# AdrianHeath988/orion

Hardware: AMD Instinct MI355X
Metric: encrypted images/sec (LoLa N=2^15) + NTT HBM GB/s vs peak (higher is better)
Workload: dtype u64; 1 GPU; LoLA (models/lola.py) lola_n15: N=2^15, LogQ=[60]+[40]x11, LogP=[60,60], input level 5, Standard ring; batch_per_gpu=64, global_batch=64

## Files before the change

orion_amd/csrc/backend.hip:

```cpp
#include <hip/hip_runtime.h>
#include <math.h>
#include <string.h>

#include <algorithm>
#include <atomic>
#include <map>
#include <memory>
#include <mutex>
#include <set>
#include <shared_mutex>
#include <stdexcept>
#include <string>
#include <thread>
#include <unordered_map>
#include <vector>
#include <complex>

#include "../../include/orion_hip.h"
#include "common.h"
#include "hostmath.h"
#include "wire.h"

int orion_launch_ntt(int logN, const LimbSet& s, const DeviceTables* tb, bool inverse, hipStream_t st);
int orion_launch_ntt_io(int logN, const NttIO& io, const DeviceTables* tb, bool inverse, hipStream_t st);
int orion_launch_ntt2(int logN, const NttIO& io, const DeviceTables* tb, bool inverse, hipStream_t st);
int orion_launch_ntt2s(int logN, const NttIO& io, const DeviceTables* tb, bool inverse, hipStream_t st,
                       bool rows_only = false);
int orion_ntt_init();
int orion_launch_ew(int op, const LimbSet& o, const LimbSet& a, const LimbSet& b, const u64* s, const u64* ss,
                    const DeviceTables* tb, int N, hipStream_t st);
int orion_launch_tensor(const LimbSet& d, const LimbSet& a, const LimbSet& b, const DeviceTables* tb, int N,
                        hipStream_t st);
int orion_launch_gather(u64* dst, long long d_comp, long long d_limb, int nimg, int nlimb, const GatherTable& T,
                        int N, hipStream_t st);
int orion_launch_basis_ext(const LimbSet& out, const LimbSet& in, const BasisExtTable* T, const DeviceTables* tb,
                           int N, hipStream_t st);
int orion_launch_modup_all(const LimbSet& D, const LimbSet& in, const BasisExtTable* Ts, int beta, int K,
                           int nqp, const DeviceTables* tb, int N, hipStream_t st);
int orion_launch_ks_mac(const LimbSet& out, const LimbSet& D, const LimbSet& own, const MacGroups& G, int ngroup,
                        int beta, const DeviceTables* tb, int N, hipStream_t st);
int orion_launch_automorph(const LimbSet& o, const LimbSet& a, const u32* idx, const DeviceTables* tb, int N,
                           int accumulate, hipStream_t st);
int orion_launch_lt_bsgs(const LimbSet& t0, const LimbSet& t1, const LimbSet& D, const LimbSet& ct,
                         const LtBabies& Bb, const LtPlan* plan, int g0, int g1, int accumulate, const LimbSet& ptl,
                         const DeviceTables* tb, int N, hipStream_t st);
int orion_launch_lt_giant(const LimbSet& acc, const LimbSet& D, const LimbSet& own, const LimbSet& t0,
                          const LimbSet& z, const LtGiants& G, const DeviceTables* tb, int N, hipStream_t st);

int orion_launch_encode(const float* vals, int nvals, int B, double2* v, const double2* tw_inv, int logn, bool ci,
                        const LimbSet& out, double scale, const DeviceTables* tb, hipStream_t st);
int orion_launch_decode(const LimbSet& x, const u64* garner, double scale, int logn, bool ci, double2* v,
// ... 267 lines not shown
  long long limb_stride() const { return (long long)B * N; }
  long long comp_stride() const { return (long long)nlimb * B * N; }
};

struct EvKey {
  Poly k;
  int level = 0;
};

struct Ciphertext {
  Poly poly;
  int level = 0;
  long double scale = 1;
  std::string poison;
  std::shared_ptr<char> share;
};

struct Plaintext {
  Poly poly;
  int level = 0;
  long double scale = 1;
  bool qp = false;
};

struct LinTrans {
  int level = 0, N1 = 1;
  float ratio = 1;
  std::vector<int> idx;
  std::map<int, Plaintext> diags;
  std::map<int, Poly> sdiags;
// ... 35 lines not shown
  }
  static Hook& hook() {
    static Hook h = nullptr;
    return h;
  }
  using Hold = void (*)(const T&);
  static Hold& hold() {
    static Hold h = nullptr;
    return h;
  }
  using Check = void (*)(const T&);
  static Check& check() {
    static Check c = nullptr;
    return c;
  }
  int add(T&& v) {
    std::lock_guard<std::mutex> lk(mu_);
    int id;
    if (!free_.empty()) {
      id = *free_.begin();
      free_.erase(free_.begin());
    } else {
      id = next_++;
    }
    map_[id] = Entry{std::make_unique<T>(std::move(v)), g_birth.fetch_add(1), false};
    if (born) born->insert(id);
    return id;
  }
  std::set<int>* born = nullptr;
  T& get(int id) {
    const int own = id >> kCtxShift;
    if (id >= 0 && own != (base_ >> kCtxShift)) {
      HandlePool* o = resolver() ? resolver()(own) : nullptr;
      if (!o || o == this) throw std::runtime_error("handle not found: " + std::to_string(id));
      unsigned long long birth = 0;
      T& v = o->get_local(id, &birth, true);
      if (check()) check()(v);
      if (hook()) hook()(own, birth);
      if (hold()) hold()(v);
      return v;
    }
    T& v = get_local(id, nullptr);
    if (check()) check()(v);
    return v;
  }
  void touch(int id) {
    const int own = id >> kCtxShift;
    HandlePool* o = this;
    if (id >= 0 && own != (base_ >> kCtxShift)) o = resolver() ? resolver()(own) : nullptr;
    if (!o) throw std::runtime_error("handle not found: " + std::to_string(id));
    std::lock_guard<std::mutex> lk(o->mu_);
    auto it = o->map_.find(id);
    if (it != o->map_.end()) it->second.birth = g_birth.fetch_add(1);
// ... 106 lines not shown
  DeviceTables* d_tb = nullptr;
  std::vector<void*> static_bufs;
  double2 *tw_inv = nullptr, *tw_fwd = nullptr;
  std::map<int, u64*> garner;
  Prng prng{0x0123456789abcdefull};
  EncSampler enc_sampler;

  Poly sk, pk, rlk;
  bool have_sk = false, have_pk = false, have_rlk = false;
  std::map<u64, EvKey> gks;
  std::map<u64, int> key_hint;
  std::map<u64, u32*> autidx;
  std::map<std::pair<int, int>, BasisExtTable*> betab;
  std::map<std::pair<int, int>, std::vector<int>> betab_pos;
  std::map<int, BasisExtTable*> modup_arr;

  HandlePool<Plaintext> pts;
  HandlePool<Ciphertext> cts;
  HandlePool<LinTrans> lts;

  struct GraphRec {
    hipGraph_t g = nullptr;
    hipGraphExec_t x = nullptr;
    std::vector<std::pair<void*, size_t>> pins;
    std::vector<std::shared_ptr<void>> holds;
  };
  std::set<int> capture_born;
  std::vector<std::shared_ptr<void>> capture_holds;
  std::map<int, GraphRec> graphs;
  int next_graph = 0;
// ... 15 lines not shown
      if (gr) hipGraphDestroy(gr);
    }
    for (auto& kv : graphs) {
      hipGraphExecDestroy(kv.second.x);
      hipGraphDestroy(kv.second.g);
    }
    graphs.clear();
    gks.clear();
    sk = pk = rlk = Poly();
    pts.reset();
    cts.reset();
    lts.reset();
    for (auto& kv : autidx) hipFree(kv.second);
    for (auto& kv : betab) hipFree(kv.second);
    for (auto& kv : modup_arr) hipFree(kv.second);
    for (auto& kv : garner) hipFree(kv.second);
    for (void* p : static_bufs) hipFree(p);
    if (d_tb) hipFree(d_tb);
    for (auto& r : prof_recs) {
      hipEventDestroy(r.e0);
      hipEventDestroy(r.e1);
    }
    for (auto e : ev_free) hipEventDestroy(e);
    if (own_stream && stream) hipStreamDestroy(stream);
  }

  hipEvent_t ev() {
    if (!ev_free.empty()) {
      hipEvent_t e = ev_free.back();
      ev_free.pop_back();
// ... 557 lines not shown
    }
    const u128 two64 = (u128)1 << 64;
    if (src32 && t < (1ull << 32) && (ssum + 1) * t < ((u128)1 << 63)) return BEXT_NARROW;
    if (!bext_modes) return BEXT_LAZY;
    if (ns >= 3 && src32 && t >= (1ull << 32) && t < (1ull << 61) && ssum * M30 < two64 &&
        ssum * T1 < (u128)4 * t * t)
      return BEXT_WT;
    if (ns >= 4 && src62 && t < (1ull << 31) && (u128)(ns + 1) * M30 * T1 < two64 && ssum * T1 < ((u128)1 << 96))
      return BEXT_NT;
    return BEXT_LAZY;
  }

  BasisExtTable* make_betab(const std::vector<int>& src, const std::vector<int>& dst, bool centered = false) {
    no_capture("a basis extension table");
    BasisExtTable T;
    memset(&T, 0, sizeof(T));
    T.ns = (int)src.size();
    T.nt = (int)dst.size();
    T.centered = centered && T.ns == 1 ? 1 : 0;
    T.chalf = mods[src[0]] >> 1;
    if (T.ns > ORION_MAXSRC || T.nt > ORION_MAXLIMB) throw std::runtime_error("basis extension too large");
    for (int i = 0; i < T.ns; ++i) {
      const u64 si = mods[src[i]];
      T.src_mod[i] = src[i];
      T.sq[i] = si;
      T.qhatinv[i] = hm_invmod(prod_mod(src, i, si), si);
      T.qhatinv_s[i] = hm_shoup(T.qhatinv[i], si);
      T.qf[i] = (double)si;
      T.qinv_f[i] = 1.0 / T.qf[i];
    }
// ... 11 lines not shown
      R.nSs = hm_shoup(R.nS, tm);
      for (int v = 0; v < 3; ++v) R.vS[v] = hm_mulmod((u64)v, R.nS, tm);
      R.qd = (double)tm;
      R.tinv = 1.0 / (double)tm;
      R.tinv32 = std::ldexp(R.tinv, 32);
      R.k = 64 - __builtin_clzll(tm);
      R.mu2 = R.k <= 61 ? (u64)(((u128)1 << (2 * R.k + 2)) / tm) : 0;
      R.c64 = (u64)(((u128)1 << 64) % tm);
      auto pieces = [](u64 x, u32& a, u32& b, u32& c) {
        a = (u32)(x & 0x3fffffffu), b = (u32)((x >> 30) & 0x3fffffffu), c = (u32)(x >> 60);
      };
      for (int i = 0; i < T.ns; ++i) pieces(R.qh[i], R.h0[i], R.h1[i], R.h2[i]);
      pieces(R.nS, R.n0, R.n1, R.n2);
      R.mode = T.centered ? BEXT_LAZY : bext_mode(src, T.ns, tm);
    }
    BasisExtTable* d;
    HIPCHK(hipMalloc(&d, sizeof(T)));
    h2d(d, &T, sizeof(T));
    return d;
  }
  BasisExtTable* modup_tab(int level, int digit, std::vector<int>& tpos) {
    auto key = std::make_pair(level, digit);
    auto it = betab.find(key);
    if (it != betab.end()) {
      tpos = betab_pos[key];
      return it->second;
    }
    const int lo = digit * K, hi = std::min((digit + 1) * K, level + 1);
    std::vector<int> src = iota(lo, hi), dst;
    tpos.clear();
    for (int j = 0; j <= level + K; ++j) {
      if (j >= lo && j < hi) continue;
      tpos.push_back(j);
      dst.push_back(qp_mod(level, j));
// ... 14 lines not shown
    for (int i = 0; i < beta; ++i)
      HIPCHK(hipMemcpyAsync(d + i, modup_tab(level, i, tpos), sizeof(BasisExtTable), hipMemcpyDeviceToDevice,
                             stream));
    HIPCHK(hipStreamSynchronize(stream));
    modup_arr[level] = d;
    return d;
  }
  BasisExtTable* moddown_tab(int level) {
    auto key = std::make_pair(level, -1);
    auto it = betab.find(key);
    if (it != betab.end()) return it->second;
    std::vector<int> src;
    for (int k = 0; k < K; ++k) src.push_back(L + k);
    BasisExtTable* d = make_betab(src, iota(0, level + 1));
    betab[key] = d;
    return d;
  }

  u64 galois_element(int k) const {
    return hm_powmod(5, (u64)(long long)k & (nthroot - 1), nthroot);
  }
  const u32* aut_index(u64 g) {
    auto it = autidx.find(g);
    if (it != autidx.end()) return it->second;
    no_capture("an automorphism index table");
    std::vector<u32> idx(N);
    const int logM = logN + (ci ? 1 : 0);
    const u64 mask = nthroot - 1;
    for (int j = 0; j < N; ++j) {
      const u64 t1 = 2 * hm_bitrev(j, logM) + 1;
// ... 394 lines not shown
      if (rows_done) throw std::runtime_error("moddown: rows pass done, but the fused path is not taken");
      ntt(xp, true);
      Poly ext = alloc(nc, level + 1, B);
      LimbSet le = lsq(ext, 0, nc, level);
      {
        Scope sc(this, P_BEXT, 8.0 * N * B * nc * (K + level + 1));
        if (orion_launch_basis_ext(le, xp, moddown_tab(level), d_tb, N, stream))
          throw std::runtime_error("basis_ext: unsupported source count");
      }
      NttIO io = nio(dst, le);
      epilogue(io);
      ntt_io(io, false);
    }
    if (aut_g && !scatter) automorph(out, dst, aut_g, aut_acc);
  }
  void keyswitch(const LimbSet& c, int level, int B, const Poly& key, int klvl, const Poly& out,
                 const u64* add0 = nullptr, const u64* add1 = nullptr, u64 aut_g = 0, bool aut_acc = false) {
    if (klvl < level) throw std::runtime_error("evaluation key made for a lower level");
    Poly u = alloc(2, level + 1 + K, B);
    const bool rows_q = mac_fwd_rows && moddown_rows_fusable(lsqp(u, 0, 2, level, level), level,
                                                             lsq(out, 0, 2, level), aut_g, aut_acc);
    bool fwd_rows = false;
    Poly D = decompose(c, level, B, rows_q, &fwd_rows);
    const int beta = (level + 1 + K - 1) / K;
    const LimbSet uq = lsqp(u, 0, 2, level, level), oq = lsq(out, 0, 2, level);
    const bool rows = moddown_rows_fusable(uq, level, oq, aut_g, aut_acc);
    mac_groups(uq, 0, lsqp(D, 0, beta, level, level), 0, c, 0, {key.ptr()}, {klvl}, beta, add0, 0,
               add0 ? level + 1 : 0, add1, rows ? level + 1 : 0, fwd_rows);
    moddown(uq, level, oq, aut_g, aut_acc, rows);
  }
  std::vector<u64> p_mod_q(int level) const {
    std::vector<u64> v;
    for (int j = 0; j <= level; ++j) {
      u64 P = 1;
      for (int k = 0; k < K; ++k) P = hm_mulmod(P, mods[L + k] % mods[j], mods[j]);
      v.push_back(P);
    }
    return v;
  }

  Ciphertext new_ct(int level, int B, long double scale) {
    Ciphertext c;
    c.poly = alloc(2, level + 1, B);
    c.level = level;
    c.scale = scale;
    return c;
  }
  Ciphertext clone(const Ciphertext& a) {
    Ciphertext c = new_ct(a.level, a.poly.B, a.scale);
    copy(lsq(c.poly, 0, 2, a.level), lsq(a.poly, 0, 2, a.level));
    return c;
  }
  void gather(Ciphertext& dst, const std::vector<GatherSrc>& src) {
    const int nl = dst.level + 1;
    const Poly& D = dst.poly;
    if ((int)src.size() != D.B || D.nlimb < nl) throw std::runtime_error("gather: destination shape mismatch");
    for (int b0 = 0; b0 < D.B; b0 += ORION_MAXGATHER) {
      const int n = std::min(ORION_MAXGATHER, D.B - b0);
      GatherTable T;
      memset(&T, 0, sizeof(T));
      for (int i = 0; i < n; ++i) T.src[i] = src[b0 + i];
// ... 26 lines not shown
      io.s[j] = hm_invmod(mods[l] % mods[j], mods[j]);
      io.ss[j] = hm_shoup(io.s[j], mods[j]);
    }
    (void)B;
    intt_then_fwd(nio(last, last), io, 1);
    ct.level = l - 1;
    ct.scale /= (long double)mods[l];
  }

  int batch_of(int a, int b) const {
    if (a == b || b == 1) return a;
    if (a == 1) return b;
    throw std::runtime_error("batch size mismatch");
  }

  Ciphertext mul_relin(const Ciphertext& a, const Ciphertext& b) {
    if (!have_rlk) throw std::runtime_error("relinearization key not generated");
    const int level = std::min(a.level, b.level);
    const int B = batch_of(a.poly.B, b.poly.B);
    Poly d = alloc(3, level + 1, B);
    {
      LimbSet ld = lsq(d, 0, 3, level);
      const bool square = a.poly.ptr() == b.poly.ptr();
      Scope sc(this, P_TENSOR, 8.0 * N * (level + 1) * B * (square ? 5 : 7));
      orion_launch_tensor(ld, lsq(a.poly, 0, 2, level, B), lsq(b.poly, 0, 2, level, B), d_tb, N, stream);
    }
    Ciphertext out = new_ct(level, B, a.scale * b.scale);
    keyswitch(lsq(d, 2, 1, level), level, B, rlk, L - 1, out.poly, d.ptr(), d.ptr() + d.comp_stride());
    return out;
  }

  Ciphertext rotate(const Ciphertext& a, int k) { return apply_galois(a, galois_element(k)); }
  void rotate_into(const Ciphertext& a, int k, Ciphertext& out) {
    const u64 g = galois_element(k);
    const int level = a.level, B = a.poly.B;
    const EvKey& key = galois_key(g, level);
    if (!out.poly.buf) out.poly = new_ct(level, B, a.scale).poly;
    out.level = level;
    keyswitch(lsq(a.poly, 1, 1, level), level, B, key.k, key.level, out.poly, a.poly.ptr(), nullptr, g);
  }
// ... 94 lines not shown
    }
    h2d(T.d_plan, plans.data(), nplan * sizeof(LtPlan));
    T.n_plan = nplan;
    T.plan_dirty = false;
  }
  void build_dirty_plans() {
    for (int id : lts.live()) {
      LinTrans& T = lts.get(id);
      if (!T.plan_dirty || T.giants.empty()) continue;
      bool all = true;
      for (int d : T.idx) all = all && T.diags.count(d & (slots - 1));
      if (all) build_plan(T);
    }
  }

  Ciphertext eval_lt(LinTrans& T, const Ciphertext& ct) {
    const int level = std::min(ct.level, T.level);
    const int B = ct.poly.B, nqp = level + 1 + K;
    const int beta = (level + 1 + K - 1) / K;
    if (T.giants.empty()) throw std::runtime_error("linear transform without diagonals");
    for (int d : T.idx)
      if (!T.diags.count(d & (slots - 1)))
        throw std::runtime_error("linear transform diagonal " + std::to_string(d) +
                                 " is not loaded (io_mode load: call LoadPlaintextDiagonal first)");
    if (T.plan_dirty) build_plan(T);
    const std::vector<u64> pq = p_mod_q(level);
    const int nb = (int)T.slots.size();
    const int nzb = nb - (T.slots.back() == 0 ? 1 : 0);

    Poly D = nzb > 0 ? decompose(lsq(ct.poly, 1, 1, level), level, B) : alloc(1, 1, 1);
    LimbSet dl = lsqp(D, 0, 1, level, level);
// ... 37 lines not shown
          for (int gi = p * LT_MAXG; gi < p * LT_MAXG + gcount; ++gi)
            for (int b : T.index.at(T.gorder[gi]))
              for (int s = 0; s < Bb.nb; ++s)
                if (T.slots[s0 + s] == b) ++npair;
          Scope sc(this, P_LTMAC,
                   8.0 * N * (rows * ((nzb ? beta : 0) + 2.0 + 2.0 * gcount * (s0 ? 2 : 1)) +
                              (double)nqp * (2.0 * beta * nrot + npair)));
          if (orion_launch_lt_bsgs(t0, t1, dl, ctl, Bb, T.d_plan + p, 0, gcount, s0 > 0, ptl, d_tb, N, stream))
            throw std::runtime_error("lt_bsgs launch failed");
        }
      }
    }

    Poly acc = alloc(2, nqp, B);
    LimbSet la = lsqp(acc, 0, 2, level, level);
    Ciphertext out = new_ct(level, B, ct.scale * (long double)mods[T.level]);
    const LimbSet lo = lsq(out.poly, 0, 2, level);
    const bool rows = nzg > 0 && nzg <= ORION_MAXGROUP && moddown_rows_fusable(la, level, lo, 0, false);
    LimbSet z = lsqp(Tt, ng - 1, 2, level, level);
    z.comp_stride = (long long)ng * Tt.comp_stride();
    if (nzg > 0) {
      Poly T1q = alloc(nzg, level + 1, B);
      moddown(lsqp(Tt, ng, nzg, level, level), level, lsq(T1q, 0, nzg, level));
      Poly Dg = decompose(lsq(T1q, 0, nzg, level), level, B);
      for (int g0 = 0; g0 < nzg; g0 += ORION_MAXGROUP) {
        LtGiants G;
        memset(&G, 0, sizeof(G));
        G.ng = std::min(ORION_MAXGROUP, nzg - g0);
        G.beta = beta;
        G.K = K;
        G.level = level;
        G.L = L;
        G.has_zero = (has_g0 && g0 == 0) ? 1 : 0;
// ... 17 lines not shown
        Poly part;
        if (g0 > 0) {
          part = alloc(2, nqp, B);
          a = lsqp(part, 0, 2, level, level);
        }
        const double rows = (double)nqp * B;
        Scope sc(this, P_LTGIANT, 8.0 * N * (rows * (G.ng * (beta + 1.0) + 2.0 + 2.0 * G.has_zero) +
                                          (double)nqp * 2.0 * beta * G.ng));
        if (orion_launch_lt_giant(a, dg, own, t0, z, G, d_tb, N, stream))
          throw std::runtime_error("lt_giant launch failed");
        if (g0 > 0) ew(EW_ADD, la, la, a);
      }
    } else {
      copy(la, z);
    }
    moddown(la, level, lo, 0, false, rows);
    return out;
  }

  Plaintext encode_dev(const float* dvals, int nvals, int B, int level, long double scale, bool qp) {
    const int n = slots;
    if (nvals > n) throw std::runtime_error("too many values for the slot count");
    std::vector<int> md = iota(0, level + 1);
    if (qp)
      for (int k = 0; k < K; ++k) md.push_back(L + k);
    const int nl = (int)md.size();
    Plaintext pt;
    pt.level = level;
    pt.scale = scale;
    pt.qp = qp;
    pt.poly = alloc(1, nl, B);
// ... 575 lines not shown
    if (!bt.d2s.k.buf || !bt.s2d.k.buf) gen_circuit_keys(bt);
    for (const KeyNeed& n : bt.need)
      if (n.kind == BK_GALOIS) gen_galois(n.gel, n.level);
    HIPCHK(hipStreamSynchronize(stream));
  }

  Ciphertext mul_i(const Bootstrapper& bt, const Ciphertext& a) {
    Ciphertext o = new_ct(a.level, a.poly.B, a.scale);
    LimbSet mi = ls(bt.mono_i, 0, 1, iota(0, a.level + 1), iota(0, a.level + 1), a.poly.B);
    mi.ncomp = 2;
    mi.comp_stride = 0;
    ew(EW_MUL, lsq(o.poly, 0, 2, a.level), lsq(a.poly, 0, 2, a.level), mi);
    return o;
  }
  Ciphertext lt_rescale(LinTrans& T, const Ciphertext& x) {
    Ciphertext y = eval_lt(T, x);
    rescale_inplace(y);
    y.scale = x.scale;
    return y;
  }
  Ciphertext eval_mod(const Bootstrapper& bt, const Ciphertext& u) {
    Ciphertext y = eval_poly(u, bt.cosp, bt.t0);
    for (int k = 0; k < bt.r; ++k) {
      Ciphertext t = mul_relin(y, y);
      const LimbSet lt = lsq(t.poly, 0, 2, t.level);
      ew(EW_ADD, lt, lt, lt);
      std::vector<u64> c = big_const_residues(-bt.dac[k] * t.scale, t.level);
      ew1(EW_ADDC, lsq(t.poly, 0, 1, t.level), lsq(t.poly, 0, 1, t.level), &c);
      rescale_inplace(t);
      y = std::move(t);
    }
    return y;
// ... 150 lines not shown
  HIPCHK(hipStreamWaitEvent(me.stream, e, 0));
  HIPCHK(hipEventDestroy(e));
}
static void foreign_order(int owner, unsigned long long birth, bool always) {
  Context* me = t_act;
  Context* o = slot_ctx(owner);
  if (!me || !o || o == me) return;
  if (!always && birth < me->synced[owner]) return;
  if (me->capturing)
    throw std::runtime_error("a captured op reads context " + std::to_string(owner) +
                             "'s newer object: capture on the context that owns it, or run the stream once first");
  const unsigned long long stamp = g_birth.load();
  wait_on(*me, *o);
  if (!always) me->synced[owner] = stamp;
}
static HandlePool<Ciphertext>* res_cts(int i) { Context* c = slot_ctx(i); return c ? &c->cts : nullptr; }
static HandlePool<Plaintext>* res_pts(int i) { Context* c = slot_ctx(i); return c ? &c->pts : nullptr; }
static HandlePool<LinTrans>* res_lts(int i) { Context* c = slot_ctx(i); return c ? &c->lts : nullptr; }
static HandlePool<Context::PolyFn>* res_polys(int i) { Context* c = slot_ctx(i); return c ? &c->polys : nullptr; }
static const bool g_hooks_set = [] {
  HandlePool<Ciphertext>::resolver() = res_cts;
  HandlePool<Plaintext>::resolver() = res_pts;
  HandlePool<LinTrans>::resolver() = res_lts;
  HandlePool<Context::PolyFn>::resolver() = res_polys;
  HandlePool<Ciphertext>::hook() = [](int o, unsigned long long b) { foreign_order(o, b, true); };
  HandlePool<Plaintext>::hook() = [](int o, unsigned long long b) { foreign_order(o, b, false); };
  HandlePool<LinTrans>::hook() = [](int o, unsigned long long b) { foreign_order(o, b, false); };
  HandlePool<Context::PolyFn>::hook() = [](int o, unsigned long long b) { foreign_order(o, b, false); };
  HandlePool<Ciphertext>::check() = [](const Ciphertext& c) {
    if (!c.poison.empty()) throw std::runtime_error(c.poison);
  };
  HandlePool<Ciphertext>::hold() = [](const Ciphertext& c) {
    if (t_act && t_act->capturing && c.poly.buf) t_act->capture_holds.push_back(c.poly.buf);
  };
  HandlePool<Plaintext>::hold() = [](const Plaintext& p) {
    if (t_act && t_act->capturing && p.poly.buf) t_act->capture_holds.push_back(p.poly.buf);
  };
  HandlePool<LinTrans>::hold() = [](const LinTrans& t) {
    if (!t_act || !t_act->capturing) return;
    for (auto& kv : t.diags)
      if (kv.second.poly.buf) t_act->capture_holds.push_back(kv.second.poly.buf);
    for (auto& kv : t.sdiags)
      if (kv.second.buf) t_act->capture_holds.push_back(kv.second.buf);
    if (t.plan) t_act->capture_holds.push_back(t.plan);
  };
  return true;
// ... 90 lines not shown
      "GetPlaintextScale", "GetCiphertextScaleF", "GetCiphertextLevel", "GetPlaintextLevel", "GetCiphertextSlots",
      "GetPlaintextSlots", "GetCiphertextDegree", "GetCiphertextBatch", "GetPlaintextBatch", "GetLiveCiphertexts",
      "GetLivePlaintexts", "GetModuliChain", "GaloisElement", "OrionHipGraphEnd", "OrionHipGetStream",
      "OrionHipCurrentPipeline"};
  return ok.count(fn) != 0;
}
static const bool g_debug_sync = getenv("ORION_DEBUG_SYNC") && atoi(getenv("ORION_DEBUG_SYNC")) != 0;
static void capture_guard(const char* fn) {
  Context* c = t_act;
  if (c && c->capturing && !capture_ok(fn))
    throw std::runtime_error(std::string(fn) + " is not allowed while capturing a graph");
  if (g_debug_sync && c && !c->capturing && c->stream) (void)hipStreamSynchronize(c->stream);
}
static int ct_ct_op(int i0, int i1, int op, bool inplace);
static void poison_deferred(Context& c, const Context::Deferred& d, const char* what) {
  const std::string msg = std::string("a deferred rotation by ") + std::to_string(d.k) + " failed (" + what +
                          "): this ciphertext was never written";
  for (int id : {d.r, d.kind == 2 ? d.x : -1}) {
    if (id < 0) continue;
    try {
      c.cts.get(id).poison = msg;
    } catch (const std::exception&) {
    }
  }
}
static void defer_flush() {
  if (!t_act || !t_act->dfr.kind) return;
  Context& c = *t_act;
  const Context::Deferred d = c.dfr;
  c.dfr = Context::Deferred();
  try {
    c.rotate_into(c.cts.get(d.x), d.k, c.cts.get(d.r));
    if (d.kind == 2) ct_ct_op(d.x, d.r, EW_ADD, true);
  } catch (const std::exception& e) {
    poison_deferred(c, d, e.what());
    throw;
  }
}
static bool defer_keeps(const char* fn) {
  static const std::set<std::string> keep = {
      "AddCiphertext", "DeleteCiphertext", "DeletePlaintext", "GetCiphertextScale", "GetCiphertextScaleF",
      "GetCiphertextLevel", "GetCiphertextSlots", "GetCiphertextDegree", "GetCiphertextBatch", "GetPlaintextScale",
      "GetPlaintextLevel", "GetPlaintextSlots", "GetPlaintextBatch", "GetLiveCiphertexts", "GetLivePlaintexts",
      "GetModuliChain", "GaloisElement", "OrionHipPeerSelect", "OrionHipPeerCount", "OrionHipGetStream",
      "OrionHipCurrentPipeline"};
  return keep.count(fn) != 0;
}
static void defer_gate(const char* fn) {
  if (!t_act || !t_act->dfr.kind) return;
  if (!defer_keeps(fn)) defer_flush();
}
#define API_BEGIN         \
  CallScope cs_;          \
  try {                   \
    cs_.act(thread_ctx(true)); \
    capture_guard(__func__); \
    defer_gate(__func__);
#define API_BEGIN_HANDLE(id) \
  CallScope cs_;             \
  try {                      \
    cs_.act(handle_ctx(id)); \
    capture_guard(__func__); \
    defer_gate(__func__);
#define API_BEGIN_NOCTX \
// ... 195 lines not shown
  return 0;
  API_END(-1)
}

void FreeCArray(void* p) { free(p); }

void DeletePlaintext(int id) {
  API_BEGIN_HANDLE(id)
  ctx().pts.del(id);
  API_END_VOID
}
void DeleteCiphertext(int id) {
  API_BEGIN_HANDLE(id)
  Context& c = ctx();
  const Context::Deferred d = c.dfr;
  if (d.kind && id == d.r) {
    c.dfr = Context::Deferred();
    if (d.kind == 2) {
      try {
        c.rotate_add_inplace(c.cts.get(d.x), d.k);
      } catch (const std::exception& e) {
        poison_deferred(c, d, e.what());
        c.cts.del(id);
        throw;
      }
    }
  } else if (d.kind && id == d.x) {
    try {
      defer_flush();
    } catch (const std::exception&) {
      c.cts.del(id);
// ... 345 lines not shown
  r.level = a.level;
  r.scale = a.scale;
  r.poly.B = a.poly.B;
  const int rid = c.cts.add(std::move(r));
  c.dfr = Context::Deferred{1, id, rid, k};
  return rid;
  API_END(-1)
}
int OrionHipRotateAdd(int id, int k) {
  API_BEGIN
  Context& c = ctx();
  c.rotate_add_inplace(c.inplace_ct(id), k);
  return id;
  API_END(-1)
}
int Rescale(int id) {
  API_BEGIN
  Context& c = ctx();
  c.rescale_inplace(c.inplace_ct(id));
  return id;
  API_END(-1)
}
int RescaleNew(int id) {
  API_BEGIN
  Context& c = ctx();
  Ciphertext& a = c.inplace_ct(id);
  c.rescale_inplace(a);
  return c.cts.add(c.alias(a));
  API_END(-1)
}

int ModDropCiphertext(int id) {
  API_BEGIN
  Ciphertext& a = ctx().inplace_ct(id);
  if (a.level < 1) throw std::runtime_error("cannot drop the last modulus");
  a.level -= 1;
  return id;
  API_END(-1)
}

static Ciphertext add_scalar(Context& c, const Ciphertext& a, float v, bool inplace_target, Ciphertext* dst) {
  (void)inplace_target;
// ... 183 lines not shown
  API_END(-1)
}
int MulRelinCiphertext(int a, int b) {
  API_BEGIN
  Context& c = ctx();
  c.inplace_ct(a, false);
  Ciphertext r = c.mul_relin(c.cts.get(a), c.cts.get(b));
  if (r.poly.B != c.cts.get(a).poly.B) throw std::runtime_error("in-place op cannot grow the batch");
  c.cts.get(a) = std::move(r);
  return a;
  API_END(-1)
}
int MulRelinCiphertextNew(int a, int b) {
  API_BEGIN
  Context& c = ctx();
  return c.cts.add(c.mul_relin(c.cts.get(a), c.cts.get(b)));
  API_END(-1)
}

void NewLinearTransformEvaluator(void) {}

static void bsgs_split(int rot, int slots, int N1, int* giant, int* baby) {
  rot &= (slots - 1);
  *giant = ((rot / N1) * N1) & (slots - 1);
  *baby = rot & (N1 - 1);
}
static int find_best_n1(const std::vector<int>& idx, int slots, int logMaxRatio) {
  const double maxRatio = (double)(1 << logMaxRatio);
  for (int N1 = 1; N1 < slots; N1 <<= 1) {
    std::set<int> gs, bs;
    for (int d : idx) {
// ... 58 lines not shown
  API_BEGIN_HANDLE(id)
  return ctx().lts.get(id).N1;
  API_END(-1)
}

int EvaluateLinearTransform(int tid, int cid) {
  API_BEGIN
  Context& c = ctx();
  LinTrans& T = c.lts.get(tid);
  Context* o = handle_ctx(tid);
  if (T.plan_dirty && o && o != &c) {
    if (o->index > c.index) throw std::runtime_error("linear transform " + std::to_string(tid) + " of pipeline " + std::to_string(o->index) + " has no device plan yet: evaluate it there first");
    std::lock_guard<std::recursive_mutex> lk(o->mu);
    if (T.plan_dirty) o->build_plan(T);
  }
  return c.cts.add(c.eval_lt(T, c.cts.get(cid)));
  API_END(-1)
}
void DeleteLinearTransform(int id) {
  API_BEGIN_HANDLE(id)
  ctx().lts.del(id);
  API_END_VOID
}
ArrayResultInt GetLinearTransformRotationKeys(int id) {
  ArrayResultInt r{nullptr, 0};
  API_BEGIN
  Context& c = ctx();
  const LinTrans& T = c.lts.get(id);
  std::vector<int> rots(T.giants.begin(), T.giants.end());
  for (int b : T.babies)
    if (std::find(rots.begin(), rots.end(), b) == rots.end()) rots.push_back(b);
// ... 875 lines not shown
```

orion_amd/csrc/common.h:

```cpp
#pragma once
#include <hip/hip_runtime.h>
#include <stdint.h>

typedef uint64_t u64;
typedef uint32_t u32;

#define ORION_MAXMOD 80
#ifndef ORION_MAXLIMB
#define ORION_MAXLIMB 64
#endif

struct ModConst {
  u64 q;
  u64 bar_mu;
  int bar_k;
  int f64;
  u64 bar_mu2;
  u64 bar_mu8;
  u64 bar_mu3;
  u64 ninv, ninv_s;
  double qd, qinv_d, ninv_d;
  u64 ciw, ciw_s;
  u64 wl, wl_s;
  double wl_d;
// ... 112 lines not shown
  u64 qhs[ORION_MAXSRC];
  u32 h0[ORION_MAXSRC], h1[ORION_MAXSRC], h2[ORION_MAXSRC];
};
struct BasisExtTable {
  int ns, nt;
  int centered;
  int pad0;
  u64 chalf;
  int src_mod[ORION_MAXSRC];
  int dst_mod[ORION_MAXLIMB];
  u64 sq[ORION_MAXSRC];
  u64 qhatinv[ORION_MAXSRC], qhatinv_s[ORION_MAXSRC];
  double qinv_f[ORION_MAXSRC];
  double qf[ORION_MAXSRC];
  BextTarget tgt[ORION_MAXLIMB];
};

#define ORION_MAXGROUP 64
__host__ __device__ static inline int key_pos(int m, int L, int klvl) { return m < L ? m : klvl + 1 + (m - L); }

struct MacGroups {
  const u64* key[ORION_MAXGROUP];
  int klvl[ORION_MAXGROUP];
  int L;
  long long out_gstride, d_gstride, add_gstride, own_gstride;
  const u64* add0;
  int K;
  int add_nq;
  const u64* add1;
  u64 add_s[ORION_MAXLIMB], add_ss[ORION_MAXLIMB];
// ... 453 lines not shown
```

orion_amd/csrc/kernels.hip:

```cpp
#include <type_traits>

#include "common.h"
#include "ntt2s_rows.h"

#ifndef LT_ABLATE
#define LT_ABLATE 0
#endif
#ifndef KS_MAC_ACC
#define KS_MAC_ACC 0
#endif
#ifndef KS_CH
#define KS_CH 2
#endif
#ifndef LT_GIANT_ACC
#define LT_GIANT_ACC 1
#endif
#ifndef LT_INT_ACC8
#define LT_INT_ACC8 1
#endif
#ifndef LT_WAVES8
#define LT_WAVES8 4
#endif
#ifndef LT_INT30
#define LT_INT30 1
// ... 146 lines not shown
  if (n >= N) return;
  const int ns = T->ns, nt = T->nt;
  u64 x0[MS], x1[MS], y0[MS], y1[MS];
#pragma unroll
  for (int i = 0; i < MS; ++i) {
    if (i >= ns) break;
    const ulonglong2 v = *(const ulonglong2*)(in.p + row_off(in, c, i, bi) + n);
    x0[i] = v.x;
    x1[i] = v.y;
  }
  const u64 v0 = bext_prep<MS>(T, x0, y0), v1 = bext_prep<MS>(T, x1, y1);
  const int tend = min(nt, (int)(blockIdx.z + 1) * tchunk);
  for (int t = blockIdx.z * tchunk; t < tend; ++t) {
    u64 o0, o1;
    bext_target2<MS>(T->tgt + t, ns, y0, v0, y1, v1, o0, o1);
    *(ulonglong2*)(out.p + row_off(out, c, t, bi) + n) = make_ulonglong2(o0, o1);
  }
}

template <int MS>
__global__ void __launch_bounds__(256) modup_all_kernel(LimbSet D, LimbSet in, const BasisExtTable* __restrict__ Ts,
                                                        int beta, int K, int nqp, int N, int tchunk) {
  const int row = blockIdx.y;
  const int bi = row % D.nbatch;
  const int r = row / D.nbatch;
  const int i = r % beta;
  const int c = r / beta;
  const int n = (blockIdx.x * kBlk + threadIdx.x) * 2;
  if (n >= N) return;
  const BasisExtTable* __restrict__ T = Ts + i;
// ... 690 lines not shown
  dim3 g = ew_grid(N, rows);
  const int nt = out.nlimb;
  g.z = target_chunks(g, nt);
  const int tc = (nt + g.z - 1) / g.z;
  if (in.nlimb <= 2)
    hipLaunchKernelGGL(basis_ext_kernel<2>, g, dim3(256), 0, st, out, in, T, N, tc);
  else if (in.nlimb <= 4)
    hipLaunchKernelGGL(basis_ext_kernel<4>, g, dim3(256), 0, st, out, in, T, N, tc);
  else if (in.nlimb <= ORION_MAXSRC)
    hipLaunchKernelGGL(basis_ext_kernel<ORION_MAXSRC>, g, dim3(256), 0, st, out, in, T, N, tc);
  else
    return -1;
  return 0;
}

int orion_launch_modup_all(const LimbSet& D, const LimbSet& in, const BasisExtTable* Ts, int beta, int K,
                           int nqp, const DeviceTables* tb, int N, hipStream_t st) {
  if (beta < 1 || nqp > ORION_MAXLIMB || D.ncomp != in.ncomp * beta) return -1;
  for (int j = 0; j < nqp; ++j)
    if (D.pos[j] != j) return -1;
  const int rows = D.ncomp * D.nbatch;
  dim3 g = ew_grid(N, rows);
  g.z = target_chunks(g, nqp);
  const int tc = (nqp + g.z - 1) / g.z;
  if (K <= 2)
    hipLaunchKernelGGL(modup_all_kernel<2>, g, dim3(256), 0, st, D, in, Ts, beta, K, nqp, N, tc);
  else if (K <= 4)
    hipLaunchKernelGGL(modup_all_kernel<4>, g, dim3(256), 0, st, D, in, Ts, beta, K, nqp, N, tc);
  else if (K <= ORION_MAXSRC)
    hipLaunchKernelGGL(modup_all_kernel<ORION_MAXSRC>, g, dim3(256), 0, st, D, in, Ts, beta, K, nqp, N, tc);
// ... 87 lines not shown
```

Before: 2345 images/s.

## Fuse keyswitch ModDown with the following rescale through a deferred pending QP ciphertext

MulRelin and linear-transform outputs can now keep their QP-basis accumulator as a pending result. ModDown only runs when the next operation needs it. When the next call is Rescale, a new basis-extension kernel folds the drop of the top q limb into the P-to-Q extension, so a single inverse-NTT pass and an NTT with a subtract-and-scale epilogue replace a separate moddown and rescale. This saves one round of NTTs and one memory pass per level. It adds deferred-state bookkeeping, cross-context finishing hooks and new precomputed tables, and it bypasses the existing row-fused moddown path.

```diff
diff --git a/orion_amd/csrc/backend.hip b/orion_amd/csrc/backend.hip
--- a/orion_amd/csrc/backend.hip
+++ b/orion_amd/csrc/backend.hip
@@ -35,6 +35,8 @@
                         int N, hipStream_t st);
 int orion_launch_basis_ext(const LimbSet& out, const LimbSet& in, const BasisExtTable* T, const DeviceTables* tb,
                            int N, hipStream_t st);
+int orion_launch_basis_ext_rescale(const LimbSet& out, const LimbSet& in, const BextRescaleTable* W, int N,
+                                   hipStream_t st);
 int orion_launch_modup_all(const LimbSet& D, const LimbSet& in, const BasisExtTable* Ts, int beta, int K,
                            int nqp, const DeviceTables* tb, int N, hipStream_t st);
 int orion_launch_ks_mac(const LimbSet& out, const LimbSet& D, const LimbSet& own, const MacGroups& G, int ngroup,
@@ -332,6 +334,7 @@
   long double scale = 1;
   std::string poison;
   std::shared_ptr<char> share;
+  Poly pend;
 };
 
 struct Plaintext {
@@ -397,6 +400,11 @@
     static Check c = nullptr;
     return c;
   }
+  using Fix = void (*)(T&, int owner);
+  static Fix& fix() {
+    static Fix f = nullptr;
+    return f;
+  }
   int add(T&& v) {
     std::lock_guard<std::mutex> lk(mu_);
     int id;
@@ -420,6 +428,7 @@
       T& v = o->get_local(id, &birth, true);
       if (check()) check()(v);
       if (hook()) hook()(own, birth);
+      if (fix()) fix()(v, own);
       if (hold()) hold()(v);
       return v;
     }
@@ -556,6 +565,7 @@
   std::map<std::pair<int, int>, BasisExtTable*> betab;
   std::map<std::pair<int, int>, std::vector<int>> betab_pos;
   std::map<int, BasisExtTable*> modup_arr;
+  std::map<int, BextRescaleTable*> mdrs_tab;
 
   HandlePool<Plaintext> pts;
   HandlePool<Ciphertext> cts;
@@ -601,6 +611,7 @@
     for (auto& kv : autidx) hipFree(kv.second);
     for (auto& kv : betab) hipFree(kv.second);
     for (auto& kv : modup_arr) hipFree(kv.second);
+    for (auto& kv : mdrs_tab) hipFree(kv.second);
     for (auto& kv : garner) hipFree(kv.second);
     for (void* p : static_bufs) hipFree(p);
     if (d_tb) hipFree(d_tb);
@@ -1188,6 +1199,13 @@
   BasisExtTable* make_betab(const std::vector<int>& src, const std::vector<int>& dst, bool centered = false) {
     no_capture("a basis extension table");
     BasisExtTable T;
+    fill_betab(T, src, dst, centered);
+    BasisExtTable* d;
+    HIPCHK(hipMalloc(&d, sizeof(T)));
+    h2d(d, &T, sizeof(T));
+    return d;
+  }
+  void fill_betab(BasisExtTable& T, const std::vector<int>& src, const std::vector<int>& dst, bool centered) const {
     memset(&T, 0, sizeof(T));
     T.ns = (int)src.size();
     T.nt = (int)dst.size();
@@ -1229,10 +1247,6 @@
       pieces(R.nS, R.n0, R.n1, R.n2);
       R.mode = T.centered ? BEXT_LAZY : bext_mode(src, T.ns, tm);
     }
-    BasisExtTable* d;
-    HIPCHK(hipMalloc(&d, sizeof(T)));
-    h2d(d, &T, sizeof(T));
-    return d;
   }
   BasisExtTable* modup_tab(int level, int digit, std::vector<int>& tpos) {
     auto key = std::make_pair(level, digit);
@@ -1277,6 +1291,35 @@
     for (int k = 0; k < K; ++k) src.push_back(L + k);
     BasisExtTable* d = make_betab(src, iota(0, level + 1));
     betab[key] = d;
+    return d;
+  }
+  BextRescaleTable* moddown_rescale_tab(int level) {
+    auto it = mdrs_tab.find(level);
+    if (it != mdrs_tab.end()) return it->second;
+    no_capture("a basis extension table");
+    if (level < 1 || level >= L) throw std::runtime_error("moddown_rescale: no such level");
+    std::vector<int> src;
+    for (int k = 0; k < K; ++k) src.push_back(L + k);
+    std::vector<BextRescaleTable> W(1);
+    memset(&W[0], 0, sizeof(BextRescaleTable));
+    fill_betab(W[0].bx, src, iota(0, level + 1), false);
+    const std::vector<u64> pq = p_mod_q(level);
+    const u64 ql = mods[level], h = ql >> 1;
+    W[0].piv = level;
+    W[0].pinv = hm_invmod(pq[level], ql);
+    W[0].pinvs = hm_shoup(W[0].pinv, ql);
+    W[0].h = h;
+    for (int i = 0; i < level; ++i) {
+      BextRescaleTarget& R = W[0].rt[i];
+      R.pq = pq[i];
+      R.pqs = hm_shoup(pq[i], mods[i]);
+      R.hm = h % mods[i];
+      R.ones = hm_shoup(1, mods[i]);
+    }
+    BextRescaleTable* d;
+    HIPCHK(hipMalloc(&d, sizeof(BextRescaleTable)));
+    h2d(d, W.data(), sizeof(BextRescaleTable));
+    mdrs_tab[level] = d;
     return d;
   }
 
@@ -1701,10 +1744,46 @@
     }
     if (aut_g && !scatter) automorph(out, dst, aut_g, aut_acc);
   }
+  bool moddown_rescale_ok(int nc, int B, int level) {
+    return level >= 1 && K <= ORION_MAXSRC && !fuse_bext(nc * B * (level + 1), K, NTT_EPI_SUBSCALE, false);
+  }
+  void moddown_rescale(const LimbSet& x, int level, const LimbSet& out) {
+    const int nc = x.ncomp, B = x.nbatch, l = level;
+    if (l < 1) throw std::runtime_error("cannot rescale a level-0 ciphertext");
+    if (out.nlimb != l) throw std::runtime_error("moddown_rescale: the output has level - 1");
+    BextRescaleTable* W = moddown_rescale_tab(l);
+    LimbSet xs = limbs(x, l, K + 1);
+    ntt(xs, true);
+    Poly ext = alloc(nc, l, B);
+    LimbSet le = lsq(ext, 0, nc, l - 1);
+    {
+      Scope sc(this, P_BEXT, 8.0 * N * B * nc * (K + 1 + l));
+      if (orion_launch_basis_ext_rescale(le, xs, W, N, stream))
+        throw std::runtime_error("basis_ext: unsupported source count");
+    }
+    NttIO io = nio(out, le);
+    io.epi = NTT_EPI_SUBSCALE;
+    io.ex = limbs(x, 0, l);
+    const std::vector<u64> pq = p_mod_q(l - 1);
+    for (int j = 0; j < l; ++j) {
+      io.s[j] = hm_invmod(hm_mulmod(pq[j], mods[l] % mods[j], mods[j]), mods[j]);
+      io.ss[j] = hm_shoup(io.s[j], mods[j]);
+    }
+    ntt_io(io, false);
+  }
   void keyswitch(const LimbSet& c, int level, int B, const Poly& key, int klvl, const Poly& out,
-                 const u64* add0 = nullptr, const u64* add1 = nullptr, u64 aut_g = 0, bool aut_acc = false) {
+                 const u64* add0 = nullptr, const u64* add1 = nullptr, u64 aut_g = 0, bool aut_acc = false,
+                 Poly* keep_qp = nullptr) {
     if (klvl < level) throw std::runtime_error("evaluation key made for a lower level");
     Poly u = alloc(2, level + 1 + K, B);
+    if (keep_qp) {
+      Poly D = decompose(c, level, B);
+      const int beta = (level + 1 + K - 1) / K;
+      mac_groups(lsqp(u, 0, 2, level, level), 0, lsqp(D, 0, beta, level, level), 0, c, 0, {key.ptr()}, {klvl}, beta,
+                 add0, 0, add0 ? level + 1 : 0, add1, 0, false);
+      *keep_qp = u;
+      return;
+    }
     const bool rows_q = mac_fwd_rows && moddown_rows_fusable(lsqp(u, 0, 2, level, level), level,
                                                              lsq(out, 0, 2, level), aut_g, aut_acc);
     bool fwd_rows = false;
@@ -1732,6 +1811,30 @@
     c.level = level;
     c.scale = scale;
     return c;
+  }
+  Ciphertext pending_ct(int level, int B, long double scale) {
+    Ciphertext c;
+    c.poly.B = B;
+    c.level = level;
+    c.scale = scale;
+    return c;
+  }
+  void finish_moddown(Ciphertext& r) {
+    if (!r.pend.buf) return;
+    const int B = r.pend.B;
+    Poly o = alloc(2, r.level + 1, B);
+    moddown(lsqp(r.pend, 0, 2, r.level, r.level), r.level, lsq(o, 0, 2, r.level));
+    r.poly = o;
+    r.pend = Poly();
+  }
+  void finish_moddown_rescale(Ciphertext& r) {
+    const int l = r.level, B = r.pend.B;
+    Poly o = alloc(2, l, B);
+    moddown_rescale(lsqp(r.pend, 0, 2, l, l), l, lsq(o, 0, 2, l - 1));
+    r.poly = o;
+    r.pend = Poly();
+    r.level = l - 1;
+    r.scale /= (long double)mods[l];
   }
   Ciphertext clone(const Ciphertext& a) {
     Ciphertext c = new_ct(a.level, a.poly.B, a.scale);
@@ -1788,7 +1891,7 @@
     throw std::runtime_error("batch size mismatch");
   }
 
-  Ciphertext mul_relin(const Ciphertext& a, const Ciphertext& b) {
+  Ciphertext mul_relin(const Ciphertext& a, const Ciphertext& b, bool keep_qp = false) {
     if (!have_rlk) throw std::runtime_error("relinearization key not generated");
     const int level = std::min(a.level, b.level);
     const int B = batch_of(a.poly.B, b.poly.B);
@@ -1798,6 +1901,12 @@
       const bool square = a.poly.ptr() == b.poly.ptr();
       Scope sc(this, P_TENSOR, 8.0 * N * (level + 1) * B * (square ? 5 : 7));
       orion_launch_tensor(ld, lsq(a.poly, 0, 2, level, B), lsq(b.poly, 0, 2, level, B), d_tb, N, stream);
+    }
+    if (keep_qp && moddown_rescale_ok(2, B, level)) {
+      Ciphertext out = pending_ct(level, B, a.scale * b.scale);
+      keyswitch(lsq(d, 2, 1, level), level, B, rlk, L - 1, out.poly, d.ptr(), d.ptr() + d.comp_stride(), 0, false,
+                &out.pend);
+      return out;
     }
     Ciphertext out = new_ct(level, B, a.scale * b.scale);
     keyswitch(lsq(d, 2, 1, level), level, B, rlk, L - 1, out.poly, d.ptr(), d.ptr() + d.comp_stride());
@@ -1922,7 +2031,7 @@
     }
   }
 
-  Ciphertext eval_lt(LinTrans& T, const Ciphertext& ct) {
+  Ciphertext eval_lt(LinTrans& T, const Ciphertext& ct, bool keep_qp = false) {
     const int level = std::min(ct.level, T.level);
     const int B = ct.poly.B, nqp = level + 1 + K;
     const int beta = (level + 1 + K - 1) / K;
@@ -1990,9 +2099,12 @@
 
     Poly acc = alloc(2, nqp, B);
     LimbSet la = lsqp(acc, 0, 2, level, level);
-    Ciphertext out = new_ct(level, B, ct.scale * (long double)mods[T.level]);
-    const LimbSet lo = lsq(out.poly, 0, 2, level);
-    const bool rows = nzg > 0 && nzg <= ORION_MAXGROUP && moddown_rows_fusable(la, level, lo, 0, false);
+    const bool pend = keep_qp && moddown_rescale_ok(2, B, level);
+    Ciphertext out = pend ? pending_ct(level, B, ct.scale * (long double)mods[T.level])
+                          : new_ct(level, B, ct.scale * (long double)mods[T.level]);
+    const LimbSet lo = pend ? la : lsq(out.poly, 0, 2, level);
+    const bool rows =
+        !pend && nzg > 0 && nzg <= ORION_MAXGROUP && moddown_rows_fusable(la, level, lo, 0, false);
     LimbSet z = lsqp(Tt, ng - 1, 2, level, level);
     z.comp_stride = (long long)ng * Tt.comp_stride();
     if (nzg > 0) {
@@ -2040,7 +2152,10 @@
     } else {
       copy(la, z);
     }
-    moddown(la, level, lo, 0, false, rows);
+    if (pend)
+      out.pend = acc;
+    else
+      moddown(la, level, lo, 0, false, rows);
     return out;
   }
 
@@ -2646,8 +2761,11 @@
     return o;
   }
   Ciphertext lt_rescale(LinTrans& T, const Ciphertext& x) {
-    Ciphertext y = eval_lt(T, x);
-    rescale_inplace(y);
+    Ciphertext y = eval_lt(T, x, defer_on);
+    if (y.pend.buf)
+      finish_moddown_rescale(y);
+    else
+      rescale_inplace(y);
     y.scale = x.scale;
     return y;
   }
@@ -2828,6 +2946,18 @@
   wait_on(*me, *o);
   if (!always) me->synced[owner] = stamp;
 }
+static void foreign_finish(Ciphertext& v, int owner) {
+  Context* me = t_act;
+  Context* o = slot_ctx(owner);
+  if (!v.pend.buf || !me || !o || o == me) return;
+  const int level = v.level;
+  Poly out = o->alloc(2, level + 1, v.pend.B);
+  wait_on(*me, *o);
+  me->moddown(me->lsqp(v.pend, 0, 2, level, level), level, me->lsq(out, 0, 2, level));
+  wait_on(*o, *me);
+  v.poly = out;
+  v.pend = Poly();
+}
 static HandlePool<Ciphertext>* res_cts(int i) { Context* c = slot_ctx(i); return c ? &c->cts : nullptr; }
 static HandlePool<Plaintext>* res_pts(int i) { Context* c = slot_ctx(i); return c ? &c->pts : nullptr; }
 static HandlePool<LinTrans>* res_lts(int i) { Context* c = slot_ctx(i); return c ? &c->lts : nullptr; }
@@ -2844,6 +2974,7 @@
   HandlePool<Ciphertext>::check() = [](const Ciphertext& c) {
     if (!c.poison.empty()) throw std::runtime_error(c.poison);
   };
+  HandlePool<Ciphertext>::fix() = foreign_finish;
   HandlePool<Ciphertext>::hold() = [](const Ciphertext& c) {
     if (t_act && t_act->capturing && c.poly.buf) t_act->capture_holds.push_back(c.poly.buf);
   };
@@ -2964,8 +3095,9 @@
 }
 static int ct_ct_op(int i0, int i1, int op, bool inplace);
 static void poison_deferred(Context& c, const Context::Deferred& d, const char* what) {
-  const std::string msg = std::string("a deferred rotation by ") + std::to_string(d.k) + " failed (" + what +
-                          "): this ciphertext was never written";
+  const std::string msg = (d.kind == 3 ? std::string("a deferred ModDown")
+                                       : std::string("a deferred rotation by ") + std::to_string(d.k)) +
+                          " failed (" + what + "): this ciphertext was never written";
   for (int id : {d.r, d.kind == 2 ? d.x : -1}) {
     if (id < 0) continue;
     try {
@@ -2980,6 +3112,10 @@
   const Context::Deferred d = c.dfr;
   c.dfr = Context::Deferred();
   try {
+    if (d.kind == 3) {
+      c.finish_moddown(c.cts.get(d.r));
+      return;
+    }
     c.rotate_into(c.cts.get(d.x), d.k, c.cts.get(d.r));
     if (d.kind == 2) ct_ct_op(d.x, d.r, EW_ADD, true);
   } catch (const std::exception& e) {
@@ -2998,6 +3134,7 @@
 }
 static void defer_gate(const char* fn) {
   if (!t_act || !t_act->dfr.kind) return;
+  if (t_act->dfr.kind == 3 && (!strcmp(fn, "Rescale") || !strcmp(fn, "RescaleNew"))) return;
   if (!defer_keeps(fn)) defer_flush();
 }
 #define API_BEGIN         \
@@ -3223,7 +3360,9 @@
   API_BEGIN_HANDLE(id)
   Context& c = ctx();
   const Context::Deferred d = c.dfr;
-  if (d.kind && id == d.r) {
+  if (d.kind == 3) {
+    if (id == d.r) c.dfr = Context::Deferred();
+  } else if (d.kind && id == d.r) {
     c.dfr = Context::Deferred();
     if (d.kind == 2) {
       try {
@@ -3599,18 +3738,39 @@
   return id;
   API_END(-1)
 }
+static Ciphertext& rescale_handle(Context& c, int id) {
+  const Context::Deferred d = c.dfr;
+  if (d.kind != 3 || d.r != id) {
+    defer_flush();
+    Ciphertext& a = c.inplace_ct(id);
+    c.rescale_inplace(a);
+    return a;
+  }
+  Ciphertext& a = c.inplace_ct(id);
+  c.dfr = Context::Deferred();
+  if (!a.pend.buf) {
+    c.rescale_inplace(a);
+    return a;
+  }
+  try {
+    c.finish_moddown_rescale(a);
+  } catch (const std::exception& e) {
+    poison_deferred(c, d, e.what());
+    throw;
+  }
+  return a;
+}
 int Rescale(int id) {
   API_BEGIN
   Context& c = ctx();
-  c.rescale_inplace(c.inplace_ct(id));
+  rescale_handle(c, id);
   return id;
   API_END(-1)
 }
 int RescaleNew(int id) {
   API_BEGIN
   Context& c = ctx();
-  Ciphertext& a = c.inplace_ct(id);
-  c.rescale_inplace(a);
+  Ciphertext& a = rescale_handle(c, id);
   return c.cts.add(c.alias(a));
   API_END(-1)
 }
@@ -3824,7 +3984,11 @@
 int MulRelinCiphertextNew(int a, int b) {
   API_BEGIN
   Context& c = ctx();
-  return c.cts.add(c.mul_relin(c.cts.get(a), c.cts.get(b)));
+  Ciphertext r = c.mul_relin(c.cts.get(a), c.cts.get(b), c.defer_on);
+  const bool pend = (bool)r.pend.buf;
+  const int rid = c.cts.add(std::move(r));
+  if (pend) c.dfr = Context::Deferred{3, -1, rid, 0};
+  return rid;
   API_END(-1)
 }
 
@@ -3913,7 +4077,11 @@
     std::lock_guard<std::recursive_mutex> lk(o->mu);
     if (T.plan_dirty) o->build_plan(T);
   }
-  return c.cts.add(c.eval_lt(T, c.cts.get(cid)));
+  Ciphertext r = c.eval_lt(T, c.cts.get(cid), c.defer_on);
+  const bool pend = (bool)r.pend.buf;
+  const int rid = c.cts.add(std::move(r));
+  if (pend) c.dfr = Context::Deferred{3, -1, rid, 0};
+  return rid;
   API_END(-1)
 }
 void DeleteLinearTransform(int id) {
diff --git a/orion_amd/csrc/common.h b/orion_amd/csrc/common.h
--- a/orion_amd/csrc/common.h
+++ b/orion_amd/csrc/common.h
@@ -150,6 +150,18 @@
   double qinv_f[ORION_MAXSRC];
   double qf[ORION_MAXSRC];
   BextTarget tgt[ORION_MAXLIMB];
+};
+struct BextRescaleTarget {
+  u64 pq, pqs;
+  u64 hm;
+  u64 ones;
+};
+struct BextRescaleTable {
+  BasisExtTable bx;
+  int piv, pad;
+  u64 pinv, pinvs;
+  u64 h;
+  BextRescaleTarget rt[ORION_MAXLIMB];
 };
 
 #define ORION_MAXGROUP 64
diff --git a/orion_amd/csrc/kernels.hip b/orion_amd/csrc/kernels.hip
--- a/orion_amd/csrc/kernels.hip
+++ b/orion_amd/csrc/kernels.hip
@@ -184,6 +184,48 @@
   for (int t = blockIdx.z * tchunk; t < tend; ++t) {
     u64 o0, o1;
     bext_target2<MS>(T->tgt + t, ns, y0, v0, y1, v1, o0, o1);
+    *(ulonglong2*)(out.p + row_off(out, c, t, bi) + n) = make_ulonglong2(o0, o1);
+  }
+}
+
+template <int MS>
+__global__ void __launch_bounds__(256) basis_ext_rescale_kernel(LimbSet out, LimbSet in,
+                                                                const BextRescaleTable* __restrict__ W, int N,
+                                                                int tchunk) {
+  const int row = blockIdx.y;
+  const int bi = row % out.nbatch;
+  const int c = row / out.nbatch;
+  const int n = (blockIdx.x * kBlk + threadIdx.x) * 2;
+  if (n >= N) return;
+  const BasisExtTable* __restrict__ T = &W->bx;
+  const int ns = T->ns, piv = W->piv;
+  u64 x0[MS], x1[MS], y0[MS], y1[MS];
+#pragma unroll
+  for (int i = 0; i < MS; ++i) {
+    if (i >= ns) break;
+    const ulonglong2 v = *(const ulonglong2*)(in.p + row_off(in, c, 1 + i, bi) + n);
+    x0[i] = v.x;
+    x1[i] = v.y;
+  }
+  const u64 v0 = bext_prep<MS>(T, x0, y0), v1 = bext_prep<MS>(T, x1, y1);
+  u64 r0, r1;
+  {
+    const ulonglong2 xl = *(const ulonglong2*)(in.p + row_off(in, c, 0, bi) + n);
+    const u64 ql = T->tgt[piv].q, pinv = W->pinv, pinvs = W->pinvs, h = W->h;
+    u64 e0, e1;
+    bext_target2<MS>(T->tgt + piv, ns, y0, v0, y1, v1, e0, e1);
+    r0 = add_mod(shoup_mul(sub_mod(xl.x, e0, ql), pinv, pinvs, ql), h, ql);
+    r1 = add_mod(shoup_mul(sub_mod(xl.y, e1, ql), pinv, pinvs, ql), h, ql);
+  }
+  const int tend = min(piv, (int)(blockIdx.z + 1) * tchunk);
+  for (int t = blockIdx.z * tchunk; t < tend; ++t) {
+    u64 o0, o1;
+    bext_target2<MS>(T->tgt + t, ns, y0, v0, y1, v1, o0, o1);
+    const BextRescaleTarget* __restrict__ R = W->rt + t;
+    const u64 q = T->tgt[t].q, pq = R->pq, pqs = R->pqs, hm = R->hm, ones = R->ones;
+    const u64 t0 = sub_mod(shoup_mul(r0, 1, ones, q), hm, q), t1 = sub_mod(shoup_mul(r1, 1, ones, q), hm, q);
+    o0 = add_mod(o0, shoup_mul(t0, pq, pqs, q), q);
+    o1 = add_mod(o1, shoup_mul(t1, pq, pqs, q), q);
     *(ulonglong2*)(out.p + row_off(out, c, t, bi) + n) = make_ulonglong2(o0, o1);
   }
 }
@@ -904,6 +946,25 @@
   return 0;
 }
 
+int orion_launch_basis_ext_rescale(const LimbSet& out, const LimbSet& in, const BextRescaleTable* W, int N,
+                                   hipStream_t st) {
+  const int rows = out.ncomp * out.nbatch, ns = in.nlimb - 1;
+  if (out.nlimb < 1 || ns < 1 || in.ncomp != out.ncomp || in.nbatch != out.nbatch) return -1;
+  dim3 g = ew_grid(N, rows);
+  const int nt = out.nlimb;
+  g.z = target_chunks(g, nt);
+  const int tc = (nt + g.z - 1) / g.z;
+  if (ns <= 2)
+    hipLaunchKernelGGL(basis_ext_rescale_kernel<2>, g, dim3(256), 0, st, out, in, W, N, tc);
+  else if (ns <= 4)
+    hipLaunchKernelGGL(basis_ext_rescale_kernel<4>, g, dim3(256), 0, st, out, in, W, N, tc);
+  else if (ns <= ORION_MAXSRC)
+    hipLaunchKernelGGL(basis_ext_rescale_kernel<ORION_MAXSRC>, g, dim3(256), 0, st, out, in, W, N, tc);
+  else
+    return -1;
+  return 0;
+}
+
 int orion_launch_modup_all(const LimbSet& D, const LimbSet& in, const BasisExtTable* Ts, int beta, int K,
                            int nqp, const DeviceTables* tb, int N, hipStream_t st) {
   if (beta < 1 || nqp > ORION_MAXLIMB || D.ncomp != in.ncomp * beta) return -1;
```

Measured after the change: 2406 images/s, median of 6. 2.6% higher.
